# yassouali/pytorch-segmentation

Measured on NVIDIA H100. Metric: images/sec DeepLabV3+/ResNet101 513x513 train step (fwd+CE+bwd+SGD), higher is better.
Workload: dtype bf16

## Files before the change

### pytorch-segmentation_b200/csrc/seg_conv_tc.cu

```cuda
#include <cuda.h>
#include <mutex>
#include <stdlib.h>
#include "seg_common.cuh"
#include "seg_ptx.cuh"
#include "seg_sync.cuh"

namespace seg {
namespace tc {

using namespace ptx;

constexpr int BM = 128;
constexpr int BK = 64;
constexpr int A_BYTES = BM * 128;
constexpr int KIND_KK = 0, KIND_KM = 1, KIND_MM = 2;
constexpr int NTHREADS = 384;
constexpr int NCONS = 256;
constexpr int MAXT = 49;

struct TcParams {
  CUtensorMap mapA;
  CUtensorMap mapB;
  int M;
  int Ncols;
  int taps;
  int kchunks;
  int stride;
  int lower_h, lower_w;
  int PQ, Q;
  int x_im2col;
  int brows_per_tap;
  short tap_wt[MAXT];
  short tap_oh[MAXT];
  short tap_ow[MAXT];
  void* out;
  long long ldo;
  int out_dtype;
  float beta;
  const float* bias;
  double* stats;
  unsigned* stat_ticket;
  SyncDesc sync;
  int out_strided, out_H, out_W, osy, osx, opy, opx;
  int kblocks_total, kblocks_per_split;
  float* dw;
  int dw_K, dw_C;
  float* ws;
};

template <int BN>
struct Cfg {
  static constexpr int B_BYTES = BN * 128;
  static constexpr int STAGE_BYTES = A_BYTES + B_BYTES;
  static constexpr int STAGES = BN == 64 ? 6 : (BN == 128 ? 5 : 4);
  static constexpr int STAT_BYTES = 2 * 2 * BN * 4;
  static constexpr int SMEM = STAGES * STAGE_BYTES + STAT_BYTES + 1024  + 256 ;
  static_assert(STAGES * STAGE_BYTES >= BM * BN * 4, "staging tile must fit in the pipeline ring");
  static_assert(SMEM <= 227 * 1024, "shared memory per block");
};

__device__ __forceinline__ void row_to_coords(int m, int PQ, int Q, int stride, int lower_h, int lower_w, int& n, int& h,
                                              int& w) {
  n = m / PQ;
  int rem = m - n * PQ;
  int pp = rem / Q;
  int qq = rem - pp * Q;
  h = lower_h + pp * stride;
  w = lower_w + qq * stride;
}

template <int BN, int TA, int TB>
__device__ __forceinline__ void wgmma_tile(float* acc, uint64_t adesc, uint64_t bdesc, uint32_t accumulate) {
  if constexpr (BN == 64) wgmma_m64n64k16<TA, TB>(acc, adesc, bdesc, accumulate);
  else if constexpr (BN == 128) wgmma_m64n128k16<TA, TB>(acc, adesc, bdesc, accumulate);
  else wgmma_m64n256k16<TA, TB>(acc, adesc, bdesc, accumulate);
}

__device__ __forceinline__ void consumer_sync() { asm volatile("bar.sync 1, 256;" ::: "memory"); }

template <int BN, int KIND>
__global__ void __launch_bounds__(NTHREADS, 1) conv_gemm_tc(const __grid_constant__ TcParams p) {
  using C = Cfg<BN>;
  constexpr int STAGES = C::STAGES;
  extern __shared__ uint8_t smem_raw[];
  const uint32_t raw_addr = smem_u32(smem_raw);
  const uint32_t smem0 = (raw_addr + 1023u) & ~1023u;
  uint8_t* smem_gen = smem_raw + (smem0 - raw_addr);
  float* stat_sm = reinterpret_cast<float*>(smem_gen + STAGES * C::STAGE_BYTES);
  const uint32_t bar0 = smem0 + STAGES * C::STAGE_BYTES + C::STAT_BYTES;
  auto full_bar = [&](int s) { return bar0 + 8u * s; };
  auto empty_bar = [&](int s) { return bar0 + 8u * (STAGES + s); };
  volatile int* flag_sm = reinterpret_cast<volatile int*>(smem_gen + STAGES * C::STAGE_BYTES + C::STAT_BYTES + 8 * 2 * STAGES);

  const int m0 = blockIdx.x * BM;
  const int n0 = blockIdx.y * BN;

  int tap_mm = 0, kb_begin = 0, kb_end = 0, num_iters;
  if (KIND == KIND_MM) {
    tap_mm = blockIdx.z % p.taps;
    const int split = blockIdx.z / p.taps;
    kb_begin = split * p.kblocks_per_split;
    kb_end = min(kb_begin + p.kblocks_per_split, p.kblocks_total);
    num_iters = max(kb_end - kb_begin, 0);
  } else {
    num_iters = p.taps * p.kchunks;
  }

  if (threadIdx.x == 0) {
    prefetch_tmap(&p.mapA);
    prefetch_tmap(&p.mapB);
    for (int s = 0; s < STAGES; ++s) {
      mbar_init(full_bar(s), 1);
      mbar_init(empty_bar(s), 8);
    }
    fence_mbar_init();
  }
  __syncthreads();
  pdl_wait();

  if (threadIdx.x < 128) {
    if (threadIdx.x == 0 && num_iters > 0) {
      if (KIND != KIND_MM) {
        int n_img = 0, h0 = 0, w0 = 0;
        if (p.x_im2col) row_to_coords(m0, p.PQ, p.Q, p.stride, p.lower_h, p.lower_w, n_img, h0, w0);
        int it = 0;
        for (int tap = 0; tap < p.taps; ++tap) {
          const int wtap = p.tap_wt[tap];
          const uint16_t oh = (uint16_t)p.tap_oh[tap], ow = (uint16_t)p.tap_ow[tap];
          for (int kc = 0; kc < p.kchunks; ++kc, ++it) {
            const int st = it % STAGES;
            const uint32_t ph = (it / STAGES) & 1;
            mbar_wait_nocall(empty_bar(st), ph ^ 1u);
            const uint32_t a_dst = smem0 + st * C::STAGE_BYTES;
            const uint32_t b_dst = a_dst + A_BYTES;
            mbar_arrive_expect_tx(full_bar(st), C::STAGE_BYTES);
            if (p.x_im2col)
              tma_load_im2col_4d(a_dst, &p.mapA, full_bar(st), kc * BK, w0, h0, n_img, ow, oh);
            else
              tma_load_2d(a_dst, &p.mapA, full_bar(st), kc * BK, m0);
            if (KIND == KIND_KK) {
              tma_load_2d(b_dst, &p.mapB, full_bar(st), kc * BK, wtap * p.brows_per_tap + n0);
            } else {
#pragma unroll
              for (int j = 0; j < BN / 64; ++j)
                tma_load_2d(b_dst + j * 8192, &p.mapB, full_bar(st), n0 + j * 64, wtap * p.brows_per_tap + kc * BK);
            }
          }
        }
      } else {
        const uint16_t oh = (uint16_t)p.tap_oh[tap_mm], ow = (uint16_t)p.tap_ow[tap_mm];
        int it = 0;
        for (int kb = kb_begin; kb < kb_end; ++kb, ++it) {
          const int st = it % STAGES;
          const uint32_t ph = (it / STAGES) & 1;
          mbar_wait_nocall(empty_bar(st), ph ^ 1u);
          const uint32_t a_dst = smem0 + st * C::STAGE_BYTES;
          const uint32_t b_dst = a_dst + A_BYTES;
          const int pix0 = kb * BK;
          mbar_arrive_expect_tx(full_bar(st), C::STAGE_BYTES);
          tma_load_2d(a_dst, &p.mapA, full_bar(st), m0, pix0);
          tma_load_2d(a_dst + 8192, &p.mapA, full_bar(st), m0 + 64, pix0);
          if (p.x_im2col) {
            int n_img, h0, w0;
            row_to_coords(pix0, p.PQ, p.Q, p.stride, p.lower_h, p.lower_w, n_img, h0, w0);
#pragma unroll
            for (int j = 0; j < BN / 64; ++j)
              tma_load_im2col_4d(b_dst + j * 8192, &p.mapB, full_bar(st), n0 + j * 64, w0, h0, n_img, ow, oh);
          } else {
#pragma unroll
            for (int j = 0; j < BN / 64; ++j) tma_load_2d(b_dst + j * 8192, &p.mapB, full_bar(st), n0 + j * 64, pix0);
          }
        }
      }
    }
    return;
  }

  if (KIND == KIND_MM && num_iters == 0) return;
  const int ctid = threadIdx.x - 128;
  const int cw = ctid >> 7;
  const int warp = (ctid >> 5) & 3, lane = ctid & 31;
  float acc[BN / 2];
#pragma unroll
  for (int i = 0; i < BN / 2; ++i) acc[i] = 0.f;
  {
    constexpr int TA = (KIND == KIND_MM) ? 1 : 0;
    constexpr int TB = (KIND == KIND_KK) ? 0 : 1;
    for (int it = 0; it < num_iters; ++it) {
      const int st = it % STAGES;
      mbar_wait_nocall(full_bar(st), (it / STAGES) & 1);
      const uint32_t a_addr = smem0 + st * C::STAGE_BYTES + cw * 8192;
      const uint32_t b_addr = smem0 + st * C::STAGE_BYTES + A_BYTES;
      const uint64_t adesc0 = make_smem_desc_sw128(a_addr, TA ? 8192 : 16, 1024);
      const uint64_t bdesc0 = make_smem_desc_sw128(b_addr, TB ? 8192 : 16, 1024);
      wgmma_fence();
#pragma unroll
      for (int k = 0; k < BK / 16; ++k) {
        const uint64_t adesc = adesc0 + (uint64_t)(TA ? (k * 2048 >> 4) : (k * 32 >> 4));
        const uint64_t bdesc = bdesc0 + (uint64_t)(TB ? (k * 2048 >> 4) : (k * 32 >> 4));
        wgmma_tile<BN, TA, TB>(acc, adesc, bdesc, 1u);
      }
      wgmma_commit();
      wgmma_wait<1>();
      __syncwarp();
      if (it > 0 && lane == 0) mbar_arrive(empty_bar((it - 1) % STAGES));
    }
    wgmma_wait<0>();
  }
  consumer_sync();

  const bool out_f32 = (KIND == KIND_MM) || p.out_dtype != SEG_DT_BF16;
  const int esize = out_f32 ? 4 : 2;
  const int CPR = BN * esize / 16;
  const int swz = (CPR >= 32 ? 31 : CPR - 1);
  uint8_t* stage = smem_gen;
  const int ncols_tile = min(BN, p.Ncols - n0);
  {
    const int r0 = cw * 64 + warp * 16 + (lane >> 2);
#pragma unroll
    for (int j = 0; j < BN / 8; ++j) {
      const int col = j * 8 + 2 * (lane & 3);
      float b0 = 0.f, b1 = 0.f;
      if (KIND != KIND_MM && p.bias) {
        if (col < ncols_tile) b0 = __ldg(p.bias + n0 + col);
        if (col + 1 < ncols_tile) b1 = __ldg(p.bias + n0 + col + 1);
      }
#pragma unroll
      for (int h = 0; h < 2; ++h) {
        const int r = r0 + 8 * h;
        const float x0 = acc[4 * j + 2 * h] + b0, x1 = acc[4 * j + 2 * h + 1] + b1;
        const int byte = col * esize;
        uint8_t* dst = stage + (size_t)r * (BN * esize) + ((((byte >> 4) ^ (r & swz))) << 4) + (byte & 15);
        if (out_f32)
          *reinterpret_cast<float2*>(dst) = make_float2(x0, x1);
        else
          *reinterpret_cast<__nv_bfloat162*>(dst) = __floats2bfloat162_rn(x0, x1);
      }
    }
  }
  consumer_sync();

  if (KIND == KIND_MM) {
    float* base = p.ws ? p.ws + (size_t)(blockIdx.z / p.taps) * p.taps * p.dw_K * p.dw_C : p.dw;
    for (int idx = ctid; idx < BM * CPR; idx += NCONS) {
      const int tr = idx / CPR, c16 = idx - tr * CPR;
      const int row = m0 + tr, col0 = c16 * 4;
      if (row >= p.M || col0 >= ncols_tile) continue;
      const float4 v = *reinterpret_cast<const float4*>(stage + (size_t)tr * (BN * 4) + ((c16 ^ (tr & swz)) << 4));
      float* dst = base + ((size_t)tap_mm * p.dw_K + row) * p.dw_C + n0 + col0;
      const bool vec = col0 + 4 <= ncols_tile && ((reinterpret_cast<uintptr_t>(dst) & 15) == 0);
      const float a[4] = {v.x, v.y, v.z, v.w};
      if (p.ws) {
        if (vec)
          *reinterpret_cast<float4*>(dst) = v;
        else
          for (int i = 0; i < 4; ++i)
            if (col0 + i < ncols_tile) dst[i] = a[i];
      } else if (vec) {
        asm volatile("red.global.add.v4.f32 [%0], {%1, %2, %3, %4};" ::"l"(dst), "f"(v.x), "f"(v.y), "f"(v.z), "f"(v.w)
                     : "memory");
      } else {
        for (int i = 0; i < 4; ++i)
          if (col0 + i < ncols_tile) atomicAdd(dst + i, a[i]);
      }
    }
    return;
  }

  if (p.stats) {
    constexpr int NG = NCONS / BN, RPG = BM / NG;
    const int c = ctid % BN, g = ctid / BN;
    const int rend = min((g + 1) * RPG, p.M - m0);
    float s1 = 0.f, s2 = 0.f;
    const int byte = c * esize;
    for (int r = g * RPG; r < rend; ++r) {
      const uint8_t* src = stage + (size_t)r * (BN * esize) + ((((byte >> 4) ^ (r & swz))) << 4) + (byte & 15);
      const float x = out_f32 ? *reinterpret_cast<const float*>(src) : bf2f(*reinterpret_cast<const __nv_bfloat16*>(src));
      s1 += x;
      s2 = fmaf(x, x, s2);
    }
    stat_sm[(g * 2 + 0) * BN + c] = s1;
    stat_sm[(g * 2 + 1) * BN + c] = s2;
  }

  {
    const int nchunks = (ncols_tile * esize + 15) >> 4;
    const bool vec_ok = ((p.ldo * esize) & 15) == 0 && ((reinterpret_cast<uintptr_t>(p.out) + (size_t)n0 * esize) & 15) == 0;
    for (int idx = ctid; idx < BM * CPR; idx += NCONS) {
      const int tr = idx / CPR;
      const int c16 = idx - tr * CPR;
      if (c16 >= nchunks) continue;
      const int grow = m0 + tr;
      if (grow >= p.M) continue;
      long long pixel = grow;
      if (p.out_strided) {
        const int n = grow / p.PQ;
        const int rem = grow - n * p.PQ;
        const int i = rem / p.Q, j = rem - i * p.Q;
        pixel = ((long long)n * p.out_H + (i * p.osy + p.opy)) * p.out_W + (j * p.osx + p.opx);
      }
      const uint8_t* src = stage + (size_t)tr * (BN * esize) + ((c16 ^ (tr & swz)) << 4);
      uint8_t* dst = reinterpret_cast<uint8_t*>(p.out) + ((size_t)pixel * p.ldo + n0) * esize + ((size_t)c16 << 4);
      const int first_col = (c16 << 4) / esize;
      const bool full = first_col + 16 / esize <= ncols_tile;
      if (!out_f32) {
        bf16x8 val = *reinterpret_cast<const bf16x8*>(src);
        if (vec_ok && full) {
          if (p.beta != 0.f) {
            float a[8], b[8];
            unpack8(val, a);
            unpack8(*reinterpret_cast<const bf16x8*>(dst), b);
#pragma unroll
            for (int k = 0; k < 8; ++k) a[k] += p.beta * b[k];
            val = pack8(a);
          }
          *reinterpret_cast<bf16x8*>(dst) = val;
        } else {
          float a[8];
          unpack8(val, a);
          __nv_bfloat16* d = reinterpret_cast<__nv_bfloat16*>(dst);
          for (int k = 0; k < 8; ++k)
            if (first_col + k < ncols_tile) {
              float o = a[k];
              if (p.beta != 0.f) o += p.beta * bf2f(d[k]);
              d[k] = f2bf(o);
            }
        }
      } else {
        const float4 val = *reinterpret_cast<const float4*>(src);
        const float a[4] = {val.x, val.y, val.z, val.w};
        float* d = reinterpret_cast<float*>(dst);
        if (vec_ok && full && p.beta == 0.f) {
          *reinterpret_cast<float4*>(d) = val;
        } else {
          for (int k = 0; k < 4; ++k)
            if (first_col + k < ncols_tile) d[k] = (p.beta != 0.f) ? a[k] + p.beta * d[k] : a[k];
        }
      }
    }
  }
  if (num_iters > 0 && ctid == 0) pdl_trigger();

  if (p.stats) {
    constexpr int NG = NCONS / BN;
    consumer_sync();
    for (int c = ctid; c < ncols_tile; c += NCONS) {
      float a = 0.f, b = 0.f;
#pragma unroll
      for (int g = 0; g < NG; ++g) {
        a += stat_sm[(g * 2 + 0) * BN + c];
        b += stat_sm[(g * 2 + 1) * BN + c];
      }
      atomicAdd(p.stats + n0 + c, (double)a);
      atomicAdd(p.stats + p.Ncols + n0 + c, (double)b);
    }
    if (p.sync.world > 0)
      sync_push_when_last<false>(p.sync, p.stats, 2 * p.Ncols, p.stat_ticket, gridDim.x * gridDim.y, ctid, NCONS,
                          [] { asm volatile("bar.sync 1, 256;" ::: "memory"); }, flag_sm);
  }
}

typedef CUresult (*EncodeTiledFn)(CUtensorMap*, CUtensorMapDataType, cuuint32_t, void*, const cuuint64_t*,
                                  const cuuint64_t*, const cuuint32_t*, const cuuint32_t*, CUtensorMapInterleave,
                                  CUtensorMapSwizzle, CUtensorMapL2promotion, CUtensorMapFloatOOBfill);
typedef CUresult (*EncodeIm2colFn)(CUtensorMap*, CUtensorMapDataType, cuuint32_t, void*, const cuuint64_t*,
                                   const cuuint64_t*, const int*, const int*, cuuint32_t, cuuint32_t,
                                   const cuuint32_t*, CUtensorMapInterleave, CUtensorMapSwizzle,
                                   CUtensorMapL2promotion, CUtensorMapFloatOOBfill);
static EncodeTiledFn g_encode_tiled = nullptr;
static EncodeIm2colFn g_encode_im2col = nullptr;
static int g_driver_version = 0;

static int resolve_driver() {
  static std::once_flag once;
  static int status = 0;
  std::call_once(once, [] {
    void* f1 = nullptr;
    void* f2 = nullptr;
    cudaDriverEntryPointQueryResult q;
    if (cudaGetDriverEntryPoint("cuTensorMapEncodeTiled", &f1, cudaEnableDefault, &q) != cudaSuccess || !f1) status = 1;
    if (cudaGetDriverEntryPoint("cuTensorMapEncodeIm2col", &f2, cudaEnableDefault, &q) != cudaSuccess || !f2) status = 1;
    g_encode_tiled = (EncodeTiledFn)f1;
    g_encode_im2col = (EncodeIm2colFn)f2;
    cudaDriverGetVersion(&g_driver_version);
  });
  if (status) set_error("cannot resolve cuTensorMapEncode* driver entry points");
  return status;
}

static int make_map_2d(CUtensorMap* m, const void* ptr, int64_t rows, int64_t cols, int64_t ld, int box_rows) {
  if (resolve_driver()) return 1;
  SEG_REQUIRE((reinterpret_cast<uintptr_t>(ptr) & 15) == 0, "TMA: base pointer not 16-byte aligned");
  SEG_REQUIRE(ld % 8 == 0, "TMA: row pitch %lld not a multiple of 8 elements", (long long)ld);
  cuuint64_t dims[2] = {(cuuint64_t)cols, (cuuint64_t)rows};
  cuuint64_t strides[1] = {(cuuint64_t)ld * 2};
  cuuint32_t box[2] = {64, (cuuint32_t)box_rows};
  cuuint32_t es[2] = {1, 1};
  CUresult r = g_encode_tiled(m, CU_TENSOR_MAP_DATA_TYPE_BFLOAT16, 2, const_cast<void*>(ptr), dims, strides, box, es,
                              CU_TENSOR_MAP_INTERLEAVE_NONE, CU_TENSOR_MAP_SWIZZLE_128B,
                              CU_TENSOR_MAP_L2_PROMOTION_L2_256B, CU_TENSOR_MAP_FLOAT_OOB_FILL_NONE);
  SEG_REQUIRE(r == CUDA_SUCCESS, "cuTensorMapEncodeTiled failed (%d) rows=%lld cols=%lld ld=%lld box_rows=%d", (int)r,
              (long long)rows, (long long)cols, (long long)ld, box_rows);
  return 0;
}

static int make_map_im2col(CUtensorMap* m, const void* ptr, int N, int H, int W, int C, int64_t ld, int lower_w,
                           int lower_h, int upper_w, int upper_h, int stride, int pixels) {
  if (resolve_driver()) return 1;
  SEG_REQUIRE((reinterpret_cast<uintptr_t>(ptr) & 15) == 0, "TMA: base pointer not 16-byte aligned");
  SEG_REQUIRE(ld % 8 == 0, "TMA: channel pitch %lld not a multiple of 8", (long long)ld);
  SEG_REQUIRE(lower_w >= -128 && upper_w >= -128 && lower_w <= 127 && upper_w <= 127 && lower_h >= -128 &&
                  upper_h >= -128 && lower_h <= 127 && upper_h <= 127,
              "im2col corner out of range");
  cuuint64_t dims[4] = {(cuuint64_t)C, (cuuint64_t)W, (cuuint64_t)H, (cuuint64_t)N};
  cuuint64_t strides[3] = {(cuuint64_t)ld * 2, (cuuint64_t)W * ld * 2, (cuuint64_t)H * W * ld * 2};
  int lo[2] = {lower_w, lower_h};
  int up[2] = {upper_w, upper_h};
  cuuint32_t es[4] = {1, (cuuint32_t)stride, (cuuint32_t)stride, 1};
  CUresult r = g_encode_im2col(m, CU_TENSOR_MAP_DATA_TYPE_BFLOAT16, 4, const_cast<void*>(ptr), dims, strides, lo, up,
                               64, (cuuint32_t)pixels, es, CU_TENSOR_MAP_INTERLEAVE_NONE, CU_TENSOR_MAP_SWIZZLE_128B,
                               CU_TENSOR_MAP_L2_PROMOTION_L2_256B, CU_TENSOR_MAP_FLOAT_OOB_FILL_NONE);
  SEG_REQUIRE(r == CUDA_SUCCESS,
              "cuTensorMapEncodeIm2col failed (%d) N=%d H=%d W=%d C=%d ld=%lld lo=(%d,%d) up=(%d,%d) s=%d", (int)r, N, H,
              W, C, (long long)ld, lower_w, lower_h, upper_w, upper_h, stride);
  if (g_driver_version <= 13010) {
    const uint64_t bytes = (uint64_t)N * H * W * ld * 2;
    if (bytes < 131072) reinterpret_cast<uint64_t*>(m)[1] &= ~(1ull << 21);
  }
  return 0;
}

template <int BN, int KIND>
static int launch_kernel(const TcParams& p, dim3 grid, cudaStream_t stream) {
  static bool attr_set = false;
  auto kfn = conv_gemm_tc<BN, KIND>;
  if (!attr_set) {
    cudaError_t e = cudaFuncSetAttribute(kfn, cudaFuncAttributeMaxDynamicSharedMemorySize, Cfg<BN>::SMEM);
    SEG_REQUIRE(e == cudaSuccess, "cudaFuncSetAttribute(smem=%d): %s", Cfg<BN>::SMEM, cudaGetErrorString(e));
    attr_set = true;
  }
  launch_pdl(kfn, grid, dim3(NTHREADS), (size_t)Cfg<BN>::SMEM, stream, p);
  return check_launch("conv_gemm_tc");
}

template <int KIND>
static int launch_bn(int bn, const TcParams& p, dim3 grid, cudaStream_t stream) {
  switch (bn) {
    case 64: return launch_kernel<64, KIND>(p, grid, stream);
    case 128: return launch_kernel<128, KIND>(p, grid, stream);
    case 256: return launch_kernel<256, KIND>(p, grid, stream);
  }
  set_error("bad BN %d", bn);
  return 1;
}

static int pick_bn(int ncols) {
  if (ncols <= 64) return 64;
  if (ncols < 256) return 128;
  const int waste = ceil_div(ncols, 256) * 256 - ncols;
  return waste < 128 ? 256 : 128;
}

bool supported(const seg_conv_desc* d) {
  if (d->C % 8 != 0 || d->ldx % 8 != 0) return false;
  if (d->R != d->S) return false;
  if (d->R * d->S > MAXT) return false;
  if (d->pad > 127 || d->dil * (d->R - 1) - d->pad > 127 || d->dil * (d->R - 1) - d->pad < -127) return false;
  if (d->stride > 8) return false;
  return true;
}

static bool is_pointwise(const seg_conv_desc* d) { return d->R == 1 && d->S == 1 && d->stride == 1 && d->pad == 0; }

int conv_fwd(const seg_conv_desc* d, const void* x, const void* w, void* y, int y_dtype, const float* bias, float beta,
             double* stats, unsigned* stat_ticket, const SyncDesc* sync, cudaStream_t stream) {
  SEG_REQUIRE(supported(d), "wgmma conv fwd: unsupported shape (C=%d ldx=%d R=%d pad=%d dil=%d)", d->C, d->ldx, d->R,
              d->pad, d->dil);
  TcParams p;
  memset(&p, 0, sizeof(p));
  const int64_t M = (int64_t)d->N * d->P * d->Q;
  SEG_REQUIRE(M < (1ll << 31), "M too large");
  p.M = (int)M;
  p.Ncols = d->K;
  p.taps = d->R * d->S;
  for (int t = 0; t < p.taps; ++t) {
    p.tap_wt[t] = (short)t;
    p.tap_oh[t] = (short)((t / d->S) * d->dil);
    p.tap_ow[t] = (short)((t % d->S) * d->dil);
  }
  p.kchunks = ceil_div(d->C, BK);
  p.stride = d->stride;
  p.lower_h = p.lower_w = -d->pad;
  p.PQ = d->P * d->Q;
  p.Q = d->Q;
  p.brows_per_tap = d->K;
  p.out = y;
  p.ldo = d->ldy;
  p.out_dtype = y_dtype;
  p.beta = beta;
  p.bias = bias;
  p.stats = stats;
  p.stat_ticket = stat_ticket;
  if (sync && stats) {
    SEG_REQUIRE(stat_ticket != nullptr, "conv fwd: SyncBN needs a zeroed ticket word");
    SEG_REQUIRE(4 * d->K <= sync->n_max, "conv fwd: 2*K = %d fp64 statistics exceed the SyncBN buffer (%d floats)", 2 * d->K, sync->n_max);
    p.sync = *sync;
  }
  const int64_t m_tiles = ceil_div64(M, BM);
  const int bn = pick_bn(d->K);
  if (is_pointwise(d)) {
    p.x_im2col = 0;
    if (make_map_2d(&p.mapA, x, M, d->C, d->ldx, BM)) return 1;
  } else {
    p.x_im2col = 1;
    const int upper = d->pad - (d->R - 1) * d->dil;
    if (make_map_im2col(&p.mapA, x, d->N, d->H, d->W, d->C, d->ldx, -d->pad, -d->pad, upper, upper, d->stride, BM)) return 1;
  }
  if (make_map_2d(&p.mapB, w, (int64_t)p.taps * d->K, d->C, d->C, bn)) return 1;
  dim3 grid((unsigned)m_tiles, (unsigned)ceil_div(d->K, bn), 1);
  return launch_bn<KIND_KK>(bn, p, grid, stream);
}

static int floordiv(int a, int b) { return (a >= 0) ? a / b : -((-a + b - 1) / b); }

int conv_dgrad(const seg_conv_desc* d, const void* dy, const void* w, void* dx, float beta, cudaStream_t stream) {
  SEG_REQUIRE(supported(d) && d->ldy % 8 == 0, "wgmma conv dgrad: unsupported shape (stride=%d K=%d ldy=%d)", d->stride,
              d->K, d->ldy);
  const int s = d->stride;
  const int bn = pick_bn(d->C);
  for (int py = 0; py < s; ++py) {
    for (int px = 0; px < s; ++px) {
      const int Hs = (d->H - py + s - 1) / s, Ws = (d->W - px + s - 1) / s;
      if (Hs <= 0 || Ws <= 0) continue;
      TcParams p;
      memset(&p, 0, sizeof(p));
      int rh[8], oh[8], nh = 0, rw[8], ow[8], nw = 0;
      for (int r = 0; r < d->R; ++r) {
        const int num = py + d->pad - r * d->dil;
        if (((num % s) + s) % s == 0) { rh[nh] = r; oh[nh] = floordiv(num, s); ++nh; }
      }
      for (int q = 0; q < d->S; ++q) {
        const int num = px + d->pad - q * d->dil;
        if (((num % s) + s) % s == 0) { rw[nw] = q; ow[nw] = floordiv(num, s); ++nw; }
      }
      int min_oh = 0, min_ow = 0;
      for (int i = 0; i < nh; ++i) min_oh = (i == 0) ? oh[i] : min(min_oh, oh[i]);
      for (int i = 0; i < nw; ++i) min_ow = (i == 0) ? ow[i] : min(min_ow, ow[i]);
      p.taps = nh * nw;
      for (int i = 0; i < nh; ++i)
        for (int j = 0; j < nw; ++j) {
          const int t = i * nw + j;
          p.tap_wt[t] = (short)(rh[i] * d->S + rw[j]);
          p.tap_oh[t] = (short)(oh[i] - min_oh);
          p.tap_ow[t] = (short)(ow[j] - min_ow);
        }
      const int64_t M = (int64_t)d->N * Hs * Ws;
      SEG_REQUIRE(M < (1ll << 31), "M too large");
      p.M = (int)M;
      p.Ncols = d->C;
      p.kchunks = ceil_div(d->K, BK);
      p.stride = 1;
      p.lower_h = min_oh;
      p.lower_w = min_ow;
      p.PQ = Hs * Ws;
      p.Q = Ws;
      p.brows_per_tap = d->K;
      p.out = dx;
      p.ldo = d->ldx;
      p.out_dtype = SEG_DT_BF16;
      p.beta = beta;
      if (s > 1) {
        p.out_strided = 1;
        p.out_H = d->H;
        p.out_W = d->W;
        p.osy = p.osx = s;
        p.opy = py;
        p.opx = px;
      }
      const int64_t m_tiles = ceil_div64(M, BM);
      if (p.taps > 0) {
        const bool plain = (s == 1 && is_pointwise(d));
        if (plain) {
          p.x_im2col = 0;
          if (make_map_2d(&p.mapA, dy, M, d->K, d->ldy, BM)) return 1;
        } else {
          p.x_im2col = 1;
          const int upper_h = Hs - d->P + min_oh, upper_w = Ws - d->Q + min_ow;
          if (make_map_im2col(&p.mapA, dy, d->N, d->P, d->Q, d->K, d->ldy, min_ow, min_oh, upper_w, upper_h, 1, BM)) return 1;
        }
        if (make_map_2d(&p.mapB, w, (int64_t)d->R * d->S * d->K, d->C, d->C, 64)) return 1;
      } else {
        if (beta != 0.f) continue;
        if (make_map_2d(&p.mapA, w, (int64_t)d->R * d->S * d->K, d->C, d->C, BM)) return 1;
        if (make_map_2d(&p.mapB, w, (int64_t)d->R * d->S * d->K, d->C, d->C, 64)) return 1;
      }
      dim3 grid((unsigned)m_tiles, (unsigned)ceil_div(d->C, bn), 1);
      if (launch_bn<KIND_KM>(bn, p, grid, stream)) return 1;
    }
  }
  return 0;
}

__global__ void wgrad_split_reduce_kernel(const float* __restrict__ ws, int splits, int64_t n, float* __restrict__ dw) {
  for (int64_t i = blockIdx.x * (int64_t)blockDim.x + threadIdx.x; i < n; i += (int64_t)gridDim.x * blockDim.x) {
    float acc = ws[i];
    for (int s = 1; s < splits; ++s) acc += ws[(size_t)s * n + i];
    dw[i] += acc;
  }
}

static void wgrad_plan(const seg_conv_desc* d, int& bn, int& splits, int& kblocks_per_split) {
  const bool wide = d->R * d->S >= 9 && d->C >= 256 && d->C % 256 == 0;
  bn = (d->C <= 64) ? 64 : (wide ? 256 : 128);
  const int kblocks_total = (int)ceil_div64((int64_t)d->N * d->P * d->Q, BK);
  const int tiles = ceil_div(d->K, BM) * ceil_div(d->C, bn) * d->R * d->S;
  splits = max(1, num_sms() / tiles);
  splits = min(splits, kblocks_total);
  splits = min(splits, 1024);
  kblocks_per_split = ceil_div(kblocks_total, splits);
  splits = ceil_div(kblocks_total, kblocks_per_split);
}

int64_t wgrad_workspace_floats(const seg_conv_desc* d) {
  if (!supported(d)) return 0;
  int bn, splits, kps;
  wgrad_plan(d, bn, splits, kps);
  return splits > 1 ? (int64_t)splits * d->R * d->S * d->K * d->C : 0;
}

int conv_wgrad(const seg_conv_desc* d, const void* dy, const void* x, float* dw, float* ws, cudaStream_t stream) {
  SEG_REQUIRE(supported(d) && d->ldy % 8 == 0, "wgmma conv wgrad: unsupported shape");
  TcParams p;
  memset(&p, 0, sizeof(p));
  const int64_t npix = (int64_t)d->N * d->P * d->Q;
  SEG_REQUIRE(npix < (1ll << 31), "too many pixels");
  p.M = d->K;
  p.Ncols = d->C;
  p.taps = d->R * d->S;
  for (int t = 0; t < p.taps; ++t) {
    p.tap_wt[t] = (short)t;
    p.tap_oh[t] = (short)((t / d->S) * d->dil);
    p.tap_ow[t] = (short)((t % d->S) * d->dil);
  }
  p.stride = d->stride;
  p.lower_h = p.lower_w = -d->pad;
  p.PQ = d->P * d->Q;
  p.Q = d->Q;
  p.dw = dw;
  p.dw_K = d->K;
  p.dw_C = d->C;
  p.kblocks_total = (int)ceil_div64(npix, BK);
  int bn, splits;
  wgrad_plan(d, bn, splits, p.kblocks_per_split);
  SEG_REQUIRE(splits == 1 || ws != nullptr, "wgmma conv wgrad: %d k-splits need the workspace (seg_conv2d_wgrad_workspace_floats)", splits);
  SEG_REQUIRE((int64_t)(splits - 1) * p.kblocks_per_split < p.kblocks_total, "wgmma conv wgrad: split %d has no k-blocks", splits - 1);
  if (splits > 1) p.ws = ws;
  if (make_map_2d(&p.mapA, dy, npix, d->K, d->ldy, 64)) return 1;
  if (is_pointwise(d)) {
    p.x_im2col = 0;
    if (make_map_2d(&p.mapB, x, npix, d->C, d->ldx, 64)) return 1;
  } else {
    p.x_im2col = 1;
    const int upper = d->pad - (d->R - 1) * d->dil;
    if (make_map_im2col(&p.mapB, x, d->N, d->H, d->W, d->C, d->ldx, -d->pad, -d->pad, upper, upper, d->stride, 64)) return 1;
  }
  SEG_REQUIRE((unsigned)(p.taps * splits) <= 65535u, "wgrad grid.z too large");
  dim3 grid((unsigned)ceil_div(d->K, BM), (unsigned)ceil_div(d->C, bn), (unsigned)(p.taps * splits));
  if (launch_bn<KIND_MM>(bn, p, grid, stream)) return 1;
  if (splits == 1) return 0;
  const int64_t n = (int64_t)p.taps * d->K * d->C;
  wgrad_split_reduce_kernel<<<(unsigned)std::min<int64_t>(ceil_div64(n, 256), (int64_t)num_sms() * 8), 256, 0, stream>>>(ws, splits, n, dw);
  return check_launch("wgrad_split_reduce");
}

}
}
```

### pytorch-segmentation_b200/csrc/seg_ptx.cuh

```cuda
#pragma once
#include <cuda.h>
#include <stdint.h>

namespace seg {
namespace ptx {

__device__ __forceinline__ uint32_t smem_u32(const void* p) { return (uint32_t)__cvta_generic_to_shared(p); }

__device__ __forceinline__ void mbar_init(uint32_t bar, uint32_t count) {
  asm volatile("mbarrier.init.shared::cta.b64 [%0], %1;" ::"r"(bar), "r"(count) : "memory");
}
__device__ __forceinline__ void fence_mbar_init() {
  asm volatile("fence.mbarrier_init.release.cluster;" ::: "memory");
}
__device__ __forceinline__ void fence_proxy_async() {
  asm volatile("fence.proxy.async.shared::cta;" ::: "memory");
}
__device__ __forceinline__ void mbar_arrive(uint32_t bar) {
  asm volatile("mbarrier.arrive.shared::cta.b64 _, [%0];" ::"r"(bar) : "memory");
}
__device__ __forceinline__ void mbar_arrive_expect_tx(uint32_t bar, uint32_t bytes) {
  asm volatile("mbarrier.arrive.expect_tx.shared::cta.b64 _, [%0], %1;" ::"r"(bar), "r"(bytes) : "memory");
}
__device__ __forceinline__ uint32_t mbar_try_wait(uint32_t bar, uint32_t parity) {
  uint32_t ok;
  asm volatile(
      "{\n\t.reg .pred p;\n\t"
      "mbarrier.try_wait.parity.shared::cta.b64 p, [%1], %2;\n\t"
      "selp.u32 %0, 1, 0, p;\n\t}"
      : "=r"(ok)
      : "r"(bar), "r"(parity)
      : "memory");
  return ok;
}
__device__ __forceinline__ void mbar_wait(uint32_t bar, uint32_t parity) {
  if (mbar_try_wait(bar, parity)) return;
  long long t0 = clock64();
  while (!mbar_try_wait(bar, parity)) {
    if (clock64() - t0 > 4000000000ll) {
      printf("seg_b200: mbarrier wait timeout (block %d,%d,%d thread %d bar %u parity %u)\n", blockIdx.x,
             blockIdx.y, blockIdx.z, threadIdx.x, bar, parity);
      __trap();
    }
  }
}

__device__ __forceinline__ void mbar_wait_nocall(uint32_t bar, uint32_t parity) {
  if (mbar_try_wait(bar, parity)) return;
  long long t0 = clock64();
  while (!mbar_try_wait(bar, parity))
    if (clock64() - t0 > 4000000000ll) __trap();
}

__device__ __forceinline__ void prefetch_tmap(const CUtensorMap* m) {
  asm volatile("prefetch.tensormap [%0];" ::"l"(reinterpret_cast<uint64_t>(m)) : "memory");
}
__device__ __forceinline__ void tma_load_2d(uint32_t dst, const CUtensorMap* m, uint32_t bar, int c0, int c1) {
  asm volatile(
      "cp.async.bulk.tensor.2d.shared::cluster.global.mbarrier::complete_tx::bytes [%0], [%1, {%3, %4}], [%2];" ::"r"(dst),
      "l"(reinterpret_cast<uint64_t>(m)), "r"(bar), "r"(c0), "r"(c1)
      : "memory");
}
__device__ __forceinline__ void tma_load_im2col_4d(uint32_t dst, const CUtensorMap* m, uint32_t bar, int c, int w,
                                                   int h, int n, uint16_t off_w, uint16_t off_h) {
  asm volatile(
      "cp.async.bulk.tensor.4d.shared::cluster.global.im2col.mbarrier::complete_tx::bytes [%0], [%1, {%3, %4, %5, "
      "%6}], [%2], {%7, %8};" ::"r"(dst),
      "l"(reinterpret_cast<uint64_t>(m)), "r"(bar), "r"(c), "r"(w), "r"(h), "r"(n), "h"(off_w), "h"(off_h)
      : "memory");
}

__device__ __forceinline__ void wgmma_fence() { asm volatile("wgmma.fence.sync.aligned;" ::: "memory"); }
__device__ __forceinline__ void wgmma_commit() { asm volatile("wgmma.commit_group.sync.aligned;" ::: "memory"); }
template <int N>
__device__ __forceinline__ void wgmma_wait() { asm volatile("wgmma.wait_group.sync.aligned %0;" ::"n"(N) : "memory"); }

__device__ __forceinline__ uint64_t make_smem_desc_sw128(uint32_t smem_addr, uint32_t lbo_bytes, uint32_t sbo_bytes) {
  uint64_t d = 0;
  d |= (uint64_t)((smem_addr & 0x3FFFFu) >> 4);
  d |= (uint64_t)((lbo_bytes >> 4) & 0x3FFFu) << 16;
  d |= (uint64_t)((sbo_bytes >> 4) & 0x3FFFu) << 32;
  d |= (uint64_t)1 << 62;
  return d;
}

template <int TA, int TB>
__device__ __forceinline__ void wgmma_m64n64k16(float* d, uint64_t adesc, uint64_t bdesc, uint32_t accumulate) {
  asm volatile(
      "{\n\t.reg .pred p;\n\tsetp.ne.b32 p, %34, 0;\n\t"
      "wgmma.mma_async.sync.aligned.m64n64k16.f32.bf16.bf16 "
      "{%0, %1, %2, %3, %4, %5, %6, %7, %8, %9, %10, %11, %12, %13, %14, %15, %16, %17, %18, %19, %20, %21, %22, %23, %24, %25, %26, %27, %28, %29, %30, %31}, %32, %33, p, 1, 1, %35, %36;\n\t}"
      : "+f"(d[0]), "+f"(d[1]), "+f"(d[2]), "+f"(d[3]), "+f"(d[4]), "+f"(d[5]), "+f"(d[6]), "+f"(d[7]), "+f"(d[8]), "+f"(d[9]), "+f"(d[10]), "+f"(d[11]), "+f"(d[12]), "+f"(d[13]), "+f"(d[14]), "+f"(d[15]), "+f"(d[16]), "+f"(d[17]), "+f"(d[18]), "+f"(d[19]), "+f"(d[20]), "+f"(d[21]), "+f"(d[22]), "+f"(d[23]), "+f"(d[24]), "+f"(d[25]), "+f"(d[26]), "+f"(d[27]), "+f"(d[28]), "+f"(d[29]), "+f"(d[30]), "+f"(d[31])
      : "l"(adesc), "l"(bdesc), "r"(accumulate), "n"(TA), "n"(TB)
      : "memory");
}

template <int TA, int TB>
__device__ __forceinline__ void wgmma_m64n128k16(float* d, uint64_t adesc, uint64_t bdesc, uint32_t accumulate) {
  asm volatile(
      "{\n\t.reg .pred p;\n\tsetp.ne.b32 p, %66, 0;\n\t"
      "wgmma.mma_async.sync.aligned.m64n128k16.f32.bf16.bf16 "
      "{%0, %1, %2, %3, %4, %5, %6, %7, %8, %9, %10, %11, %12, %13, %14, %15, %16, %17, %18, %19, %20, %21, %22, %23, %24, %25, %26, %27, %28, %29, %30, %31, %32, %33, %34, %35, %36, %37, %38, %39, %40, %41, %42, %43, %44, %45, %46, %47, %48, %49, %50, %51, %52, %53, %54, %55, %56, %57, %58, %59, %60, %61, %62, %63}, %64, %65, p, 1, 1, %67, %68;\n\t}"
      : "+f"(d[0]), "+f"(d[1]), "+f"(d[2]), "+f"(d[3]), "+f"(d[4]), "+f"(d[5]), "+f"(d[6]), "+f"(d[7]), "+f"(d[8]), "+f"(d[9]), "+f"(d[10]), "+f"(d[11]), "+f"(d[12]), "+f"(d[13]), "+f"(d[14]), "+f"(d[15]), "+f"(d[16]), "+f"(d[17]), "+f"(d[18]), "+f"(d[19]), "+f"(d[20]), "+f"(d[21]), "+f"(d[22]), "+f"(d[23]), "+f"(d[24]), "+f"(d[25]), "+f"(d[26]), "+f"(d[27]), "+f"(d[28]), "+f"(d[29]), "+f"(d[30]), "+f"(d[31]), "+f"(d[32]), "+f"(d[33]), "+f"(d[34]), "+f"(d[35]), "+f"(d[36]), "+f"(d[37]), "+f"(d[38]), "+f"(d[39]), "+f"(d[40]), "+f"(d[41]), "+f"(d[42]), "+f"(d[43]), "+f"(d[44]), "+f"(d[45]), "+f"(d[46]), "+f"(d[47]), "+f"(d[48]), "+f"(d[49]), "+f"(d[50]), "+f"(d[51]), "+f"(d[52]), "+f"(d[53]), "+f"(d[54]), "+f"(d[55]), "+f"(d[56]), "+f"(d[57]), "+f"(d[58]), "+f"(d[59]), "+f"(d[60]), "+f"(d[61]), "+f"(d[62]), "+f"(d[63])
      : "l"(adesc), "l"(bdesc), "r"(accumulate), "n"(TA), "n"(TB)
      : "memory");
}

template <int TA, int TB>
__device__ __forceinline__ void wgmma_m64n256k16(float* d, uint64_t adesc, uint64_t bdesc, uint32_t accumulate) {
  asm volatile(
      "{\n\t.reg .pred p;\n\tsetp.ne.b32 p, %130, 0;\n\t"
      "wgmma.mma_async.sync.aligned.m64n256k16.f32.bf16.bf16 "
      "{%0, %1, %2, %3, %4, %5, %6, %7, %8, %9, %10, %11, %12, %13, %14, %15, %16, %17, %18, %19, %20, %21, %22, %23, %24, %25, %26, %27, %28, %29, %30, %31, %32, %33, %34, %35, %36, %37, %38, %39, %40, %41, %42, %43, %44, %45, %46, %47, %48, %49, %50, %51, %52, %53, %54, %55, %56, %57, %58, %59, %60, %61, %62, %63, %64, %65, %66, %67, %68, %69, %70, %71, %72, %73, %74, %75, %76, %77, %78, %79, %80, %81, %82, %83, %84, %85, %86, %87, %88, %89, %90, %91, %92, %93, %94, %95, %96, %97, %98, %99, %100, %101, %102, %103, %104, %105, %106, %107, %108, %109, %110, %111, %112, %113, %114, %115, %116, %117, %118, %119, %120, %121, %122, %123, %124, %125, %126, %127}, %128, %129, p, 1, 1, %131, %132;\n\t}"
      : "+f"(d[0]), "+f"(d[1]), "+f"(d[2]), "+f"(d[3]), "+f"(d[4]), "+f"(d[5]), "+f"(d[6]), "+f"(d[7]), "+f"(d[8]), "+f"(d[9]), "+f"(d[10]), "+f"(d[11]), "+f"(d[12]), "+f"(d[13]), "+f"(d[14]), "+f"(d[15]), "+f"(d[16]), "+f"(d[17]), "+f"(d[18]), "+f"(d[19]), "+f"(d[20]), "+f"(d[21]), "+f"(d[22]), "+f"(d[23]), "+f"(d[24]), "+f"(d[25]), "+f"(d[26]), "+f"(d[27]), "+f"(d[28]), "+f"(d[29]), "+f"(d[30]), "+f"(d[31]), "+f"(d[32]), "+f"(d[33]), "+f"(d[34]), "+f"(d[35]), "+f"(d[36]), "+f"(d[37]), "+f"(d[38]), "+f"(d[39]), "+f"(d[40]), "+f"(d[41]), "+f"(d[42]), "+f"(d[43]), "+f"(d[44]), "+f"(d[45]), "+f"(d[46]), "+f"(d[47]), "+f"(d[48]), "+f"(d[49]), "+f"(d[50]), "+f"(d[51]), "+f"(d[52]), "+f"(d[53]), "+f"(d[54]), "+f"(d[55]), "+f"(d[56]), "+f"(d[57]), "+f"(d[58]), "+f"(d[59]), "+f"(d[60]), "+f"(d[61]), "+f"(d[62]), "+f"(d[63]), "+f"(d[64]), "+f"(d[65]), "+f"(d[66]), "+f"(d[67]), "+f"(d[68]), "+f"(d[69]), "+f"(d[70]), "+f"(d[71]), "+f"(d[72]), "+f"(d[73]), "+f"(d[74]), "+f"(d[75]), "+f"(d[76]), "+f"(d[77]), "+f"(d[78]), "+f"(d[79]), "+f"(d[80]), "+f"(d[81]), "+f"(d[82]), "+f"(d[83]), "+f"(d[84]), "+f"(d[85]), "+f"(d[86]), "+f"(d[87]), "+f"(d[88]), "+f"(d[89]), "+f"(d[90]), "+f"(d[91]), "+f"(d[92]), "+f"(d[93]), "+f"(d[94]), "+f"(d[95]), "+f"(d[96]), "+f"(d[97]), "+f"(d[98]), "+f"(d[99]), "+f"(d[100]), "+f"(d[101]), "+f"(d[102]), "+f"(d[103]), "+f"(d[104]), "+f"(d[105]), "+f"(d[106]), "+f"(d[107]), "+f"(d[108]), "+f"(d[109]), "+f"(d[110]), "+f"(d[111]), "+f"(d[112]), "+f"(d[113]), "+f"(d[114]), "+f"(d[115]), "+f"(d[116]), "+f"(d[117]), "+f"(d[118]), "+f"(d[119]), "+f"(d[120]), "+f"(d[121]), "+f"(d[122]), "+f"(d[123]), "+f"(d[124]), "+f"(d[125]), "+f"(d[126]), "+f"(d[127])
      : "l"(adesc), "l"(bdesc), "r"(accumulate), "n"(TA), "n"(TB)
      : "memory");
}

}
}
```

Baseline: 332.4.

## Use persistent ping-pong warp-specialized kernel for conv fprop and dgrad

Replaces the one-tile-per-block conv GEMM for forward and data-gradient convolutions with a persistent kernel sized to the SM count. In it, two consumer warpgroups alternate output tiles (ping-pong), using named barriers to order mainloops so one group's epilogue overlaps the other's MMA. Each warpgroup now computes a full 128-row tile with two accumulators, and registers are rebalanced with setmaxnreg. BN is restricted to 64/128 with fewer stages, and BN statistics grouping is parameterized. The aim is to hide epilogue and stats cost and reduce launch/tail overhead, at the cost of more register pressure and smaller tiles for wide layers.

Result: faster. 352.4, median of 6 (+6.0%).

```diff
diff --git a/pytorch-segmentation_b200/csrc/seg_conv_tc.cu b/pytorch-segmentation_b200/csrc/seg_conv_tc.cu
--- a/pytorch-segmentation_b200/csrc/seg_conv_tc.cu
+++ b/pytorch-segmentation_b200/csrc/seg_conv_tc.cu
@@ -13,10 +13,14 @@
 constexpr int BM = 128;
 constexpr int BK = 64;
 constexpr int A_BYTES = BM * 128;
-constexpr int KIND_KK = 0, KIND_KM = 1, KIND_MM = 2;
+constexpr int KIND_KK = 0, KIND_KM = 1;
 constexpr int NTHREADS = 384;
 constexpr int NCONS = 256;
 constexpr int MAXT = 49;
+
+constexpr int BAR_CONSUMERS = 1;
+constexpr int BAR_ORDER = 2;
+constexpr int BAR_WG = 4;
 
 struct TcParams {
   CUtensorMap mapA;
@@ -39,24 +43,15 @@
   float beta;
   const float* bias;
   double* stats;
+  int stat_rows;
   unsigned* stat_ticket;
   SyncDesc sync;
   int out_strided, out_H, out_W, osy, osx, opy, opx;
+  int n_tiles, tiles;
   int kblocks_total, kblocks_per_split;
   float* dw;
   int dw_K, dw_C;
   float* ws;
-};
-
-template <int BN>
-struct Cfg {
-  static constexpr int B_BYTES = BN * 128;
-  static constexpr int STAGE_BYTES = A_BYTES + B_BYTES;
-  static constexpr int STAGES = BN == 64 ? 6 : (BN == 128 ? 5 : 4);
-  static constexpr int STAT_BYTES = 2 * 2 * BN * 4;
-  static constexpr int SMEM = STAGES * STAGE_BYTES + STAT_BYTES + 1024  + 256 ;
-  static_assert(STAGES * STAGE_BYTES >= BM * BN * 4, "staging tile must fit in the pipeline ring");
-  static_assert(SMEM <= 227 * 1024, "shared memory per block");
 };
 
 __device__ __forceinline__ void row_to_coords(int m, int PQ, int Q, int stride, int lower_h, int lower_w, int& n, int& h,
@@ -76,35 +71,312 @@
   else wgmma_m64n256k16<TA, TB>(acc, adesc, bdesc, accumulate);
 }
 
-__device__ __forceinline__ void consumer_sync() { asm volatile("bar.sync 1, 256;" ::: "memory"); }
-
 template <int BN, int KIND>
-__global__ void __launch_bounds__(NTHREADS, 1) conv_gemm_tc(const __grid_constant__ TcParams p) {
+__device__ __forceinline__ void load_kblock(const TcParams& p, uint32_t a_dst, uint32_t bar, int kc, int wtap, uint16_t oh,
+                                            uint16_t ow, int n_img, int h0, int w0, int m0, int n0) {
+  const uint32_t b_dst = a_dst + A_BYTES;
+  if (p.x_im2col)
+    tma_load_im2col_4d(a_dst, &p.mapA, bar, kc * BK, w0, h0, n_img, ow, oh);
+  else
+    tma_load_2d(a_dst, &p.mapA, bar, kc * BK, m0);
+  if (KIND == KIND_KK) {
+    tma_load_2d(b_dst, &p.mapB, bar, kc * BK, wtap * p.brows_per_tap + n0);
+  } else {
+#pragma unroll
+    for (int j = 0; j < BN / 64; ++j)
+      tma_load_2d(b_dst + j * 8192, &p.mapB, bar, n0 + j * 64, wtap * p.brows_per_tap + kc * BK);
+  }
+}
+
+template <int BN>
+__device__ __forceinline__ void stage_acc(const float* acc, const float* acc1, uint8_t* stage, int rbase, int warp, int lane,
+                                          const float* bias, bool out_f32) {
+  const int esize = out_f32 ? 4 : 2;
+  const int CPR = BN * esize / 16;
+  const int swz = (CPR >= 32 ? 31 : CPR - 1);
+  const int r0 = rbase + warp * 16 + (lane >> 2);
+#pragma unroll
+  for (int j = 0; j < BN / 8; ++j) {
+    const int col = j * 8 + 2 * (lane & 3);
+    float b0 = 0.f, b1 = 0.f;
+    if (bias) {
+      b0 = bias[col];
+      b1 = bias[col + 1];
+    }
+#pragma unroll
+    for (int h = 0; h < 4; ++h) {
+      if (h >= 2 && !acc1) break;
+      const float* a = h < 2 ? acc : acc1;
+      const int r = r0 + 8 * (h & 1) + 32 * (h & 2);
+      const float x0 = a[4 * j + 2 * (h & 1)] + b0, x1 = a[4 * j + 2 * (h & 1) + 1] + b1;
+      const int byte = col * esize;
+      uint8_t* dst = stage + (size_t)r * (BN * esize) + ((((byte >> 4) ^ (r & swz))) << 4) + (byte & 15);
+      if (out_f32)
+        *reinterpret_cast<float2*>(dst) = make_float2(x0, x1);
+      else
+        *reinterpret_cast<__nv_bfloat162*>(dst) = __floats2bfloat162_rn(x0, x1);
+    }
+  }
+}
+
+
+template <int BN>
+struct PPCfg {
+  static_assert(BN == 64 || BN == 128, "ping-pong tile width");
+  static constexpr int B_BYTES = BN * 128;
+  static constexpr int STAGE_BYTES = A_BYTES + B_BYTES;
+  static constexpr int STAGES = BN == 64 ? 6 : 4;
+  static constexpr int RING = STAGES * STAGE_BYTES;
+  static constexpr int STG_BYTES = BM * 256;
+  static constexpr int MAXG = BM / 32;
+  static constexpr int STAT_BYTES = MAXG * 2 * BN * 4 + BN * 4;
+  static constexpr int SMEM = RING + 2 * (STG_BYTES + STAT_BYTES) + 1024  + 256 ;
+  static_assert(16 * STAGES + 8 <= 256, "barrier area");
+  static_assert(SMEM <= 227 * 1024, "shared memory per block");
+};
+
+template <int BN, int KIND>
+__global__ void __launch_bounds__(NTHREADS, 1) conv_gemm_pp(const __grid_constant__ TcParams p) {
+  using C = PPCfg<BN>;
+  constexpr int STAGES = C::STAGES;
+  extern __shared__ uint8_t smem_raw[];
+  const uint32_t raw_addr = smem_u32(smem_raw);
+  const uint32_t smem0 = (raw_addr + 1023u) & ~1023u;
+  uint8_t* smem_gen = smem_raw + (smem0 - raw_addr);
+  const uint32_t bar0 = smem0 + C::RING + 2 * (C::STG_BYTES + C::STAT_BYTES);
+  auto full_bar = [&](int s) { return bar0 + 8u * s; };
+  auto empty_bar = [&](int s) { return bar0 + 8u * (STAGES + s); };
+  volatile int* flag_sm = reinterpret_cast<volatile int*>(smem_gen + (bar0 - smem0) + 16 * STAGES);
+
+  const int num_iters = p.taps * p.kchunks;
+  const int grid = gridDim.x;
+  const int ntiles = (p.tiles - (int)blockIdx.x + grid - 1) / grid;
+
+  if (threadIdx.x == 0) {
+    prefetch_tmap(&p.mapA);
+    prefetch_tmap(&p.mapB);
+    for (int s = 0; s < STAGES; ++s) {
+      mbar_init(full_bar(s), 1);
+      mbar_init(empty_bar(s), 4);
+    }
+    fence_mbar_init();
+  }
+  __syncthreads();
+  pdl_wait();
+
+  if (threadIdx.x < 128) {
+    setmaxnreg_dec<40>();
+    if (threadIdx.x == 0 && num_iters > 0) {
+      int it = 0;
+      for (int j = 0; j < ntiles; ++j) {
+        const int t = blockIdx.x + j * grid;
+        const int m0 = (t / p.n_tiles) * BM, n0 = (t % p.n_tiles) * BN;
+        int n_img = 0, h0 = 0, w0 = 0;
+        if (p.x_im2col) row_to_coords(m0, p.PQ, p.Q, p.stride, p.lower_h, p.lower_w, n_img, h0, w0);
+        for (int tap = 0; tap < p.taps; ++tap) {
+          const int wtap = p.tap_wt[tap];
+          const uint16_t oh = (uint16_t)p.tap_oh[tap], ow = (uint16_t)p.tap_ow[tap];
+          for (int kc = 0; kc < p.kchunks; ++kc, ++it) {
+            const int st = it % STAGES;
+            mbar_wait_nocall(empty_bar(st), ((it / STAGES) & 1) ^ 1u);
+            mbar_arrive_expect_tx(full_bar(st), C::STAGE_BYTES);
+            load_kblock<BN, KIND>(p, smem0 + st * C::STAGE_BYTES, full_bar(st), kc, wtap, oh, ow, n_img, h0, w0, m0, n0);
+          }
+        }
+      }
+    }
+    return;
+  }
+
+  setmaxnreg_inc<232>();
+  const int cw = (threadIdx.x - 128) >> 7;
+  const int tid = threadIdx.x & 127;
+  const int warp = tid >> 5, lane = tid & 31;
+  uint8_t* stage = smem_gen + C::RING + cw * C::STG_BYTES;
+  float* stat_sm = reinterpret_cast<float*>(smem_gen + C::RING + 2 * C::STG_BYTES + cw * C::STAT_BYTES);
+  float* bias_sm = stat_sm + C::MAXG * 2 * BN;
+  const bool out_f32 = p.out_dtype != SEG_DT_BF16;
+  const int esize = out_f32 ? 4 : 2;
+  const int CPR = BN * esize / 16;
+  const int swz = (CPR >= 32 ? 31 : CPR - 1);
+  auto wg_sync = [&] { named_sync(BAR_WG + cw, 128); };
+
+  for (int j = cw; j < ntiles; j += 2) {
+    const int t = blockIdx.x + j * grid;
+    const int m0 = (t / p.n_tiles) * BM, n0 = (t % p.n_tiles) * BN;
+    float acc0[BN / 2], acc1[BN / 2];
+#pragma unroll
+    for (int i = 0; i < BN / 2; ++i) acc0[i] = acc1[i] = 0.f;
+
+    if (j > 0) named_sync(BAR_ORDER + cw, NCONS);
+    {
+      constexpr int TB = (KIND == KIND_KK) ? 0 : 1;
+      const int it0 = j * num_iters;
+      for (int i = 0; i < num_iters; ++i) {
+        const int it = it0 + i;
+        const int st = it % STAGES;
+        mbar_wait_nocall(full_bar(st), (it / STAGES) & 1);
+        const uint32_t a_addr = smem0 + st * C::STAGE_BYTES;
+        const uint32_t b_addr = a_addr + A_BYTES;
+        const uint64_t adesc0 = make_smem_desc_sw128(a_addr, 16, 1024);
+        const uint64_t adesc1 = make_smem_desc_sw128(a_addr + 8192, 16, 1024);
+        const uint64_t bdesc0 = make_smem_desc_sw128(b_addr, TB ? 8192 : 16, 1024);
+        wgmma_fence();
+#pragma unroll
+        for (int k = 0; k < BK / 16; ++k) {
+          const uint64_t bdesc = bdesc0 + (uint64_t)(TB ? (k * 2048 >> 4) : (k * 32 >> 4));
+          wgmma_tile<BN, 0, TB>(acc0, adesc0 + (uint64_t)(k * 32 >> 4), bdesc, 1u);
+          wgmma_tile<BN, 0, TB>(acc1, adesc1 + (uint64_t)(k * 32 >> 4), bdesc, 1u);
+        }
+        wgmma_commit();
+        wgmma_wait<1>();
+        __syncwarp();
+        if (i > 0 && lane == 0) mbar_arrive(empty_bar((it - 1) % STAGES));
+      }
+      if (j + 1 < ntiles) named_arrive(BAR_ORDER + (cw ^ 1), NCONS);
+      wgmma_wait<0>();
+      __syncwarp();
+      if (num_iters > 0 && lane == 0) mbar_arrive(empty_bar((it0 + num_iters - 1) % STAGES));
+    }
+
+    const int ncols_tile = min(BN, p.Ncols - n0);
+    if (p.bias && tid < BN) bias_sm[tid] = tid < ncols_tile ? __ldg(p.bias + n0 + tid) : 0.f;
+    wg_sync();
+    stage_acc<BN>(acc0, acc1, stage, 0, warp, lane, p.bias ? bias_sm : nullptr, out_f32);
+    wg_sync();
+
+    const int ngroups = BM / p.stat_rows;
+    if (p.stats) {
+      const int parts = min(128 / BN, ngroups);
+      const int rpp = BM / parts;
+      const int c = tid % BN, part = tid / BN;
+      const int rvalid = min(BM, p.M - m0);
+      if (part < parts) {
+        const int byte = c * esize;
+        int g = part * rpp / p.stat_rows;
+        for (int rg = part * rpp; rg < (part + 1) * rpp; rg += p.stat_rows, ++g) {
+          float s1 = 0.f, s2 = 0.f;
+          const int rend = min(rg + p.stat_rows, rvalid);
+          for (int r = rg; r < rend; ++r) {
+            const uint8_t* src = stage + (size_t)r * (BN * esize) + ((((byte >> 4) ^ (r & swz))) << 4) + (byte & 15);
+            const float x = out_f32 ? *reinterpret_cast<const float*>(src) : bf2f(*reinterpret_cast<const __nv_bfloat16*>(src));
+            s1 += x;
+            s2 = fmaf(x, x, s2);
+          }
+          stat_sm[(g * 2 + 0) * BN + c] = s1;
+          stat_sm[(g * 2 + 1) * BN + c] = s2;
+        }
+      }
+    }
+
+    {
+      const int nchunks = (ncols_tile * esize + 15) >> 4;
+      const bool vec_ok = ((p.ldo * esize) & 15) == 0 && ((reinterpret_cast<uintptr_t>(p.out) + (size_t)n0 * esize) & 15) == 0;
+      for (int idx = tid; idx < BM * CPR; idx += 128) {
+        const int tr = idx / CPR;
+        const int c16 = idx - tr * CPR;
+        if (c16 >= nchunks) continue;
+        const int grow = m0 + tr;
+        if (grow >= p.M) continue;
+        long long pixel = grow;
+        if (p.out_strided) {
+          const int n = grow / p.PQ;
+          const int rem = grow - n * p.PQ;
+          const int i = rem / p.Q, jj = rem - i * p.Q;
+          pixel = ((long long)n * p.out_H + (i * p.osy + p.opy)) * p.out_W + (jj * p.osx + p.opx);
+        }
+        const uint8_t* src = stage + (size_t)tr * (BN * esize) + ((c16 ^ (tr & swz)) << 4);
+        uint8_t* dst = reinterpret_cast<uint8_t*>(p.out) + ((size_t)pixel * p.ldo + n0) * esize + ((size_t)c16 << 4);
+        const int first_col = (c16 << 4) / esize;
+        const bool full = first_col + 16 / esize <= ncols_tile;
+        if (!out_f32) {
+          bf16x8 val = *reinterpret_cast<const bf16x8*>(src);
+          if (vec_ok && full) {
+            if (p.beta != 0.f) {
+              float a[8], b[8];
+              unpack8(val, a);
+              unpack8(*reinterpret_cast<const bf16x8*>(dst), b);
+#pragma unroll
+              for (int k = 0; k < 8; ++k) a[k] += p.beta * b[k];
+              val = pack8(a);
+            }
+            *reinterpret_cast<bf16x8*>(dst) = val;
+          } else {
+            float a[8];
+            unpack8(val, a);
+            __nv_bfloat16* d = reinterpret_cast<__nv_bfloat16*>(dst);
+            for (int k = 0; k < 8; ++k)
+              if (first_col + k < ncols_tile) {
+                float o = a[k];
+                if (p.beta != 0.f) o += p.beta * bf2f(d[k]);
+                d[k] = f2bf(o);
+              }
+          }
+        } else {
+          const float4 val = *reinterpret_cast<const float4*>(src);
+          const float a[4] = {val.x, val.y, val.z, val.w};
+          float* d = reinterpret_cast<float*>(dst);
+          if (vec_ok && full && p.beta == 0.f) {
+            *reinterpret_cast<float4*>(d) = val;
+          } else {
+            for (int k = 0; k < 4; ++k)
+              if (first_col + k < ncols_tile) d[k] = (p.beta != 0.f) ? a[k] + p.beta * d[k] : a[k];
+          }
+        }
+      }
+    }
+    if (j == ntiles - 1 && tid == 0) pdl_trigger();
+
+    if (p.stats) {
+      wg_sync();
+      if (tid < ncols_tile) {
+        float a = 0.f, b = 0.f;
+        for (int g = 0; g < ngroups; ++g) {
+          a += stat_sm[(g * 2 + 0) * BN + tid];
+          b += stat_sm[(g * 2 + 1) * BN + tid];
+        }
+        atomicAdd(p.stats + n0 + tid, (double)a);
+        atomicAdd(p.stats + p.Ncols + n0 + tid, (double)b);
+      }
+    }
+  }
+
+  if (p.stats && p.sync.world > 0)
+    sync_push_when_last<false>(p.sync, p.stats, 2 * p.Ncols, p.stat_ticket, gridDim.x, threadIdx.x - 128, NCONS,
+                               [] { named_sync(BAR_CONSUMERS, NCONS); }, flag_sm);
+}
+
+
+template <int BN>
+struct Cfg {
+  static constexpr int B_BYTES = BN * 128;
+  static constexpr int STAGE_BYTES = A_BYTES + B_BYTES;
+  static constexpr int STAGES = BN == 64 ? 6 : (BN == 128 ? 5 : 4);
+  static constexpr int SMEM = STAGES * STAGE_BYTES + 1024  + 256 ;
+  static_assert(STAGES * STAGE_BYTES >= BM * BN * 4, "staging tile must fit in the pipeline ring");
+  static_assert(SMEM <= 227 * 1024, "shared memory per block");
+};
+
+template <int BN>
+__global__ void __launch_bounds__(NTHREADS, 1) conv_gemm_wgrad(const __grid_constant__ TcParams p) {
   using C = Cfg<BN>;
   constexpr int STAGES = C::STAGES;
   extern __shared__ uint8_t smem_raw[];
   const uint32_t raw_addr = smem_u32(smem_raw);
   const uint32_t smem0 = (raw_addr + 1023u) & ~1023u;
   uint8_t* smem_gen = smem_raw + (smem0 - raw_addr);
-  float* stat_sm = reinterpret_cast<float*>(smem_gen + STAGES * C::STAGE_BYTES);
-  const uint32_t bar0 = smem0 + STAGES * C::STAGE_BYTES + C::STAT_BYTES;
+  const uint32_t bar0 = smem0 + STAGES * C::STAGE_BYTES;
   auto full_bar = [&](int s) { return bar0 + 8u * s; };
   auto empty_bar = [&](int s) { return bar0 + 8u * (STAGES + s); };
-  volatile int* flag_sm = reinterpret_cast<volatile int*>(smem_gen + STAGES * C::STAGE_BYTES + C::STAT_BYTES + 8 * 2 * STAGES);
 
   const int m0 = blockIdx.x * BM;
   const int n0 = blockIdx.y * BN;
 
-  int tap_mm = 0, kb_begin = 0, kb_end = 0, num_iters;
-  if (KIND == KIND_MM) {
-    tap_mm = blockIdx.z % p.taps;
-    const int split = blockIdx.z / p.taps;
-    kb_begin = split * p.kblocks_per_split;
-    kb_end = min(kb_begin + p.kblocks_per_split, p.kblocks_total);
-    num_iters = max(kb_end - kb_begin, 0);
-  } else {
-    num_iters = p.taps * p.kchunks;
-  }
+  const int tap_mm = blockIdx.z % p.taps;
+  const int split = blockIdx.z / p.taps;
+  const int kb_begin = split * p.kblocks_per_split;
+  const int kb_end = min(kb_begin + p.kblocks_per_split, p.kblocks_total);
+  const int num_iters = max(kb_end - kb_begin, 0);
 
   if (threadIdx.x == 0) {
     prefetch_tmap(&p.mapA);
@@ -120,243 +392,88 @@
 
   if (threadIdx.x < 128) {
     if (threadIdx.x == 0 && num_iters > 0) {
-      if (KIND != KIND_MM) {
-        int n_img = 0, h0 = 0, w0 = 0;
-        if (p.x_im2col) row_to_coords(m0, p.PQ, p.Q, p.stride, p.lower_h, p.lower_w, n_img, h0, w0);
-        int it = 0;
-        for (int tap = 0; tap < p.taps; ++tap) {
-          const int wtap = p.tap_wt[tap];
-          const uint16_t oh = (uint16_t)p.tap_oh[tap], ow = (uint16_t)p.tap_ow[tap];
-          for (int kc = 0; kc < p.kchunks; ++kc, ++it) {
-            const int st = it % STAGES;
-            const uint32_t ph = (it / STAGES) & 1;
-            mbar_wait_nocall(empty_bar(st), ph ^ 1u);
-            const uint32_t a_dst = smem0 + st * C::STAGE_BYTES;
-            const uint32_t b_dst = a_dst + A_BYTES;
-            mbar_arrive_expect_tx(full_bar(st), C::STAGE_BYTES);
-            if (p.x_im2col)
-              tma_load_im2col_4d(a_dst, &p.mapA, full_bar(st), kc * BK, w0, h0, n_img, ow, oh);
-            else
-              tma_load_2d(a_dst, &p.mapA, full_bar(st), kc * BK, m0);
-            if (KIND == KIND_KK) {
-              tma_load_2d(b_dst, &p.mapB, full_bar(st), kc * BK, wtap * p.brows_per_tap + n0);
-            } else {
-#pragma unroll
-              for (int j = 0; j < BN / 64; ++j)
-                tma_load_2d(b_dst + j * 8192, &p.mapB, full_bar(st), n0 + j * 64, wtap * p.brows_per_tap + kc * BK);
-            }
-          }
+      const uint16_t oh = (uint16_t)p.tap_oh[tap_mm], ow = (uint16_t)p.tap_ow[tap_mm];
+      int it = 0;
+      for (int kb = kb_begin; kb < kb_end; ++kb, ++it) {
+        const int st = it % STAGES;
+        const uint32_t ph = (it / STAGES) & 1;
+        mbar_wait_nocall(empty_bar(st), ph ^ 1u);
+        const uint32_t a_dst = smem0 + st * C::STAGE_BYTES;
+        const uint32_t b_dst = a_dst + A_BYTES;
+        const int pix0 = kb * BK;
+        mbar_arrive_expect_tx(full_bar(st), C::STAGE_BYTES);
+        tma_load_2d(a_dst, &p.mapA, full_bar(st), m0, pix0);
+        tma_load_2d(a_dst + 8192, &p.mapA, full_bar(st), m0 + 64, pix0);
+        if (p.x_im2col) {
+          int n_img, h0, w0;
+          row_to_coords(pix0, p.PQ, p.Q, p.stride, p.lower_h, p.lower_w, n_img, h0, w0);
+#pragma unroll
+          for (int j = 0; j < BN / 64; ++j)
+            tma_load_im2col_4d(b_dst + j * 8192, &p.mapB, full_bar(st), n0 + j * 64, w0, h0, n_img, ow, oh);
+        } else {
+#pragma unroll
+          for (int j = 0; j < BN / 64; ++j) tma_load_2d(b_dst + j * 8192, &p.mapB, full_bar(st), n0 + j * 64, pix0);
         }
-      } else {
-        const uint16_t oh = (uint16_t)p.tap_oh[tap_mm], ow = (uint16_t)p.tap_ow[tap_mm];
-        int it = 0;
-        for (int kb = kb_begin; kb < kb_end; ++kb, ++it) {
-          const int st = it % STAGES;
-          const uint32_t ph = (it / STAGES) & 1;
-          mbar_wait_nocall(empty_bar(st), ph ^ 1u);
-          const uint32_t a_dst = smem0 + st * C::STAGE_BYTES;
-          const uint32_t b_dst = a_dst + A_BYTES;
-          const int pix0 = kb * BK;
-          mbar_arrive_expect_tx(full_bar(st), C::STAGE_BYTES);
-          tma_load_2d(a_dst, &p.mapA, full_bar(st), m0, pix0);
-          tma_load_2d(a_dst + 8192, &p.mapA, full_bar(st), m0 + 64, pix0);
-          if (p.x_im2col) {
-            int n_img, h0, w0;
-            row_to_coords(pix0, p.PQ, p.Q, p.stride, p.lower_h, p.lower_w, n_img, h0, w0);
-#pragma unroll
-            for (int j = 0; j < BN / 64; ++j)
-              tma_load_im2col_4d(b_dst + j * 8192, &p.mapB, full_bar(st), n0 + j * 64, w0, h0, n_img, ow, oh);
-          } else {
-#pragma unroll
-            for (int j = 0; j < BN / 64; ++j) tma_load_2d(b_dst + j * 8192, &p.mapB, full_bar(st), n0 + j * 64, pix0);
-          }
-        }
       }
     }
     return;
   }
 
-  if (KIND == KIND_MM && num_iters == 0) return;
+  if (num_iters == 0) return;
   const int ctid = threadIdx.x - 128;
   const int cw = ctid >> 7;
   const int warp = (ctid >> 5) & 3, lane = ctid & 31;
   float acc[BN / 2];
 #pragma unroll
   for (int i = 0; i < BN / 2; ++i) acc[i] = 0.f;
-  {
-    constexpr int TA = (KIND == KIND_MM) ? 1 : 0;
-    constexpr int TB = (KIND == KIND_KK) ? 0 : 1;
-    for (int it = 0; it < num_iters; ++it) {
-      const int st = it % STAGES;
-      mbar_wait_nocall(full_bar(st), (it / STAGES) & 1);
-      const uint32_t a_addr = smem0 + st * C::STAGE_BYTES + cw * 8192;
-      const uint32_t b_addr = smem0 + st * C::STAGE_BYTES + A_BYTES;
-      const uint64_t adesc0 = make_smem_desc_sw128(a_addr, TA ? 8192 : 16, 1024);
-      const uint64_t bdesc0 = make_smem_desc_sw128(b_addr, TB ? 8192 : 16, 1024);
-      wgmma_fence();
-#pragma unroll
-      for (int k = 0; k < BK / 16; ++k) {
-        const uint64_t adesc = adesc0 + (uint64_t)(TA ? (k * 2048 >> 4) : (k * 32 >> 4));
-        const uint64_t bdesc = bdesc0 + (uint64_t)(TB ? (k * 2048 >> 4) : (k * 32 >> 4));
-        wgmma_tile<BN, TA, TB>(acc, adesc, bdesc, 1u);
-      }
-      wgmma_commit();
-      wgmma_wait<1>();
-      __syncwarp();
-      if (it > 0 && lane == 0) mbar_arrive(empty_bar((it - 1) % STAGES));
-    }
-    wgmma_wait<0>();
-  }
-  consumer_sync();
-
-  const bool out_f32 = (KIND == KIND_MM) || p.out_dtype != SEG_DT_BF16;
-  const int esize = out_f32 ? 4 : 2;
-  const int CPR = BN * esize / 16;
-  const int swz = (CPR >= 32 ? 31 : CPR - 1);
+  for (int it = 0; it < num_iters; ++it) {
+    const int st = it % STAGES;
+    mbar_wait_nocall(full_bar(st), (it / STAGES) & 1);
+    const uint32_t a_addr = smem0 + st * C::STAGE_BYTES + cw * 8192;
+    const uint32_t b_addr = smem0 + st * C::STAGE_BYTES + A_BYTES;
+    const uint64_t adesc0 = make_smem_desc_sw128(a_addr, 8192, 1024);
+    const uint64_t bdesc0 = make_smem_desc_sw128(b_addr, 8192, 1024);
+    wgmma_fence();
+#pragma unroll
+    for (int k = 0; k < BK / 16; ++k)
+      wgmma_tile<BN, 1, 1>(acc, adesc0 + (uint64_t)(k * 2048 >> 4), bdesc0 + (uint64_t)(k * 2048 >> 4), 1u);
+    wgmma_commit();
+    wgmma_wait<1>();
+    __syncwarp();
+    if (it > 0 && lane == 0) mbar_arrive(empty_bar((it - 1) % STAGES));
+  }
+  wgmma_wait<0>();
+  named_sync(BAR_CONSUMERS, NCONS);
+
   uint8_t* stage = smem_gen;
   const int ncols_tile = min(BN, p.Ncols - n0);
-  {
-    const int r0 = cw * 64 + warp * 16 + (lane >> 2);
-#pragma unroll
-    for (int j = 0; j < BN / 8; ++j) {
-      const int col = j * 8 + 2 * (lane & 3);
-      float b0 = 0.f, b1 = 0.f;
-      if (KIND != KIND_MM && p.bias) {
-        if (col < ncols_tile) b0 = __ldg(p.bias + n0 + col);
-        if (col + 1 < ncols_tile) b1 = __ldg(p.bias + n0 + col + 1);
-      }
-#pragma unroll
-      for (int h = 0; h < 2; ++h) {
-        const int r = r0 + 8 * h;
-        const float x0 = acc[4 * j + 2 * h] + b0, x1 = acc[4 * j + 2 * h + 1] + b1;
-        const int byte = col * esize;
-        uint8_t* dst = stage + (size_t)r * (BN * esize) + ((((byte >> 4) ^ (r & swz))) << 4) + (byte & 15);
-        if (out_f32)
-          *reinterpret_cast<float2*>(dst) = make_float2(x0, x1);
-        else
-          *reinterpret_cast<__nv_bfloat162*>(dst) = __floats2bfloat162_rn(x0, x1);
-      }
-    }
-  }
-  consumer_sync();
-
-  if (KIND == KIND_MM) {
-    float* base = p.ws ? p.ws + (size_t)(blockIdx.z / p.taps) * p.taps * p.dw_K * p.dw_C : p.dw;
-    for (int idx = ctid; idx < BM * CPR; idx += NCONS) {
-      const int tr = idx / CPR, c16 = idx - tr * CPR;
-      const int row = m0 + tr, col0 = c16 * 4;
-      if (row >= p.M || col0 >= ncols_tile) continue;
-      const float4 v = *reinterpret_cast<const float4*>(stage + (size_t)tr * (BN * 4) + ((c16 ^ (tr & swz)) << 4));
-      float* dst = base + ((size_t)tap_mm * p.dw_K + row) * p.dw_C + n0 + col0;
-      const bool vec = col0 + 4 <= ncols_tile && ((reinterpret_cast<uintptr_t>(dst) & 15) == 0);
-      const float a[4] = {v.x, v.y, v.z, v.w};
-      if (p.ws) {
-        if (vec)
-          *reinterpret_cast<float4*>(dst) = v;
-        else
-          for (int i = 0; i < 4; ++i)
-            if (col0 + i < ncols_tile) dst[i] = a[i];
-      } else if (vec) {
-        asm volatile("red.global.add.v4.f32 [%0], {%1, %2, %3, %4};" ::"l"(dst), "f"(v.x), "f"(v.y), "f"(v.z), "f"(v.w)
-                     : "memory");
-      } else {
+  stage_acc<BN>(acc, nullptr, stage, cw * 64, warp, lane, nullptr, true);
+  named_sync(BAR_CONSUMERS, NCONS);
+
+  const int CPR = BN * 4 / 16;
+  const int swz = (CPR >= 32 ? 31 : CPR - 1);
+  float* base = p.ws ? p.ws + (size_t)split * p.taps * p.dw_K * p.dw_C : p.dw;
+  for (int idx = ctid; idx < BM * CPR; idx += NCONS) {
+    const int tr = idx / CPR, c16 = idx - tr * CPR;
+    const int row = m0 + tr, col0 = c16 * 4;
+    if (row >= p.M || col0 >= ncols_tile) continue;
+    const float4 v = *reinterpret_cast<const float4*>(stage + (size_t)tr * (BN * 4) + ((c16 ^ (tr & swz)) << 4));
+    float* dst = base + ((size_t)tap_mm * p.dw_K + row) * p.dw_C + n0 + col0;
+    const bool vec = col0 + 4 <= ncols_tile && ((reinterpret_cast<uintptr_t>(dst) & 15) == 0);
+    const float a[4] = {v.x, v.y, v.z, v.w};
+    if (p.ws) {
+      if (vec)
+        *reinterpret_cast<float4*>(dst) = v;
+      else
         for (int i = 0; i < 4; ++i)
-          if (col0 + i < ncols_tile) atomicAdd(dst + i, a[i]);
-      }
-    }
-    return;
-  }
-
-  if (p.stats) {
-    constexpr int NG = NCONS / BN, RPG = BM / NG;
-    const int c = ctid % BN, g = ctid / BN;
-    const int rend = min((g + 1) * RPG, p.M - m0);
-    float s1 = 0.f, s2 = 0.f;
-    const int byte = c * esize;
-    for (int r = g * RPG; r < rend; ++r) {
-      const uint8_t* src = stage + (size_t)r * (BN * esize) + ((((byte >> 4) ^ (r & swz))) << 4) + (byte & 15);
-      const float x = out_f32 ? *reinterpret_cast<const float*>(src) : bf2f(*reinterpret_cast<const __nv_bfloat16*>(src));
-      s1 += x;
-      s2 = fmaf(x, x, s2);
-    }
-    stat_sm[(g * 2 + 0) * BN + c] = s1;
-    stat_sm[(g * 2 + 1) * BN + c] = s2;
-  }
-
-  {
-    const int nchunks = (ncols_tile * esize + 15) >> 4;
-    const bool vec_ok = ((p.ldo * esize) & 15) == 0 && ((reinterpret_cast<uintptr_t>(p.out) + (size_t)n0 * esize) & 15) == 0;
-    for (int idx = ctid; idx < BM * CPR; idx += NCONS) {
-      const int tr = idx / CPR;
-      const int c16 = idx - tr * CPR;
-      if (c16 >= nchunks) continue;
-      const int grow = m0 + tr;
-      if (grow >= p.M) continue;
-      long long pixel = grow;
-      if (p.out_strided) {
-        const int n = grow / p.PQ;
-        const int rem = grow - n * p.PQ;
-        const int i = rem / p.Q, j = rem - i * p.Q;
-        pixel = ((long long)n * p.out_H + (i * p.osy + p.opy)) * p.out_W + (j * p.osx + p.opx);
-      }
-      const uint8_t* src = stage + (size_t)tr * (BN * esize) + ((c16 ^ (tr & swz)) << 4);
-      uint8_t* dst = reinterpret_cast<uint8_t*>(p.out) + ((size_t)pixel * p.ldo + n0) * esize + ((size_t)c16 << 4);
-      const int first_col = (c16 << 4) / esize;
-      const bool full = first_col + 16 / esize <= ncols_tile;
-      if (!out_f32) {
-        bf16x8 val = *reinterpret_cast<const bf16x8*>(src);
-        if (vec_ok && full) {
-          if (p.beta != 0.f) {
-            float a[8], b[8];
-            unpack8(val, a);
-            unpack8(*reinterpret_cast<const bf16x8*>(dst), b);
-#pragma unroll
-            for (int k = 0; k < 8; ++k) a[k] += p.beta * b[k];
-            val = pack8(a);
-          }
-          *reinterpret_cast<bf16x8*>(dst) = val;
-        } else {
-          float a[8];
-          unpack8(val, a);
-          __nv_bfloat16* d = reinterpret_cast<__nv_bfloat16*>(dst);
-          for (int k = 0; k < 8; ++k)
-            if (first_col + k < ncols_tile) {
-              float o = a[k];
-              if (p.beta != 0.f) o += p.beta * bf2f(d[k]);
-              d[k] = f2bf(o);
-            }
-        }
-      } else {
-        const float4 val = *reinterpret_cast<const float4*>(src);
-        const float a[4] = {val.x, val.y, val.z, val.w};
-        float* d = reinterpret_cast<float*>(dst);
-        if (vec_ok && full && p.beta == 0.f) {
-          *reinterpret_cast<float4*>(d) = val;
-        } else {
-          for (int k = 0; k < 4; ++k)
-            if (first_col + k < ncols_tile) d[k] = (p.beta != 0.f) ? a[k] + p.beta * d[k] : a[k];
-        }
-      }
-    }
-  }
-  if (num_iters > 0 && ctid == 0) pdl_trigger();
-
-  if (p.stats) {
-    constexpr int NG = NCONS / BN;
-    consumer_sync();
-    for (int c = ctid; c < ncols_tile; c += NCONS) {
-      float a = 0.f, b = 0.f;
-#pragma unroll
-      for (int g = 0; g < NG; ++g) {
-        a += stat_sm[(g * 2 + 0) * BN + c];
-        b += stat_sm[(g * 2 + 1) * BN + c];
-      }
-      atomicAdd(p.stats + n0 + c, (double)a);
-      atomicAdd(p.stats + p.Ncols + n0 + c, (double)b);
-    }
-    if (p.sync.world > 0)
-      sync_push_when_last<false>(p.sync, p.stats, 2 * p.Ncols, p.stat_ticket, gridDim.x * gridDim.y, ctid, NCONS,
-                          [] { asm volatile("bar.sync 1, 256;" ::: "memory"); }, flag_sm);
+          if (col0 + i < ncols_tile) dst[i] = a[i];
+    } else if (vec) {
+      asm volatile("red.global.add.v4.f32 [%0], {%1, %2, %3, %4};" ::"l"(dst), "f"(v.x), "f"(v.y), "f"(v.z), "f"(v.w)
+                   : "memory");
+    } else {
+      for (int i = 0; i < 4; ++i)
+        if (col0 + i < ncols_tile) atomicAdd(dst + i, a[i]);
+    }
   }
 }
 
@@ -431,34 +548,63 @@
 }
 
 template <int BN, int KIND>
-static int launch_kernel(const TcParams& p, dim3 grid, cudaStream_t stream) {
+static int launch_pp(TcParams& p, cudaStream_t stream) {
   static bool attr_set = false;
-  auto kfn = conv_gemm_tc<BN, KIND>;
+  auto kfn = conv_gemm_pp<BN, KIND>;
+  if (!attr_set) {
+    cudaError_t e = cudaFuncSetAttribute(kfn, cudaFuncAttributeMaxDynamicSharedMemorySize, PPCfg<BN>::SMEM);
+    SEG_REQUIRE(e == cudaSuccess, "cudaFuncSetAttribute(smem=%d): %s", PPCfg<BN>::SMEM, cudaGetErrorString(e));
+    attr_set = true;
+  }
+  const int n_tiles = ceil_div(p.Ncols, BN);
+  const int64_t tiles = ceil_div64(p.M, BM) * n_tiles;
+  SEG_REQUIRE(tiles < (1ll << 31), "too many output tiles");
+  p.n_tiles = n_tiles;
+  p.tiles = (int)tiles;
+  const dim3 grid((unsigned)std::min<int64_t>(tiles, num_sms()));
+  launch_pdl(kfn, grid, dim3(NTHREADS), (size_t)PPCfg<BN>::SMEM, stream, p);
+  return check_launch("conv_gemm_pp");
+}
+
+template <int KIND>
+static int launch_pp_bn(int bn, TcParams& p, cudaStream_t stream) {
+  switch (bn) {
+    case 64: return launch_pp<64, KIND>(p, stream);
+    case 128: return launch_pp<128, KIND>(p, stream);
+  }
+  set_error("bad BN %d", bn);
+  return 1;
+}
+
+template <int BN>
+static int launch_wgrad(const TcParams& p, dim3 grid, cudaStream_t stream) {
+  static bool attr_set = false;
+  auto kfn = conv_gemm_wgrad<BN>;
   if (!attr_set) {
     cudaError_t e = cudaFuncSetAttribute(kfn, cudaFuncAttributeMaxDynamicSharedMemorySize, Cfg<BN>::SMEM);
     SEG_REQUIRE(e == cudaSuccess, "cudaFuncSetAttribute(smem=%d): %s", Cfg<BN>::SMEM, cudaGetErrorString(e));
     attr_set = true;
   }
   launch_pdl(kfn, grid, dim3(NTHREADS), (size_t)Cfg<BN>::SMEM, stream, p);
-  return check_launch("conv_gemm_tc");
-}
-
-template <int KIND>
-static int launch_bn(int bn, const TcParams& p, dim3 grid, cudaStream_t stream) {
+  return check_launch("conv_gemm_wgrad");
+}
+
+static int launch_wgrad_bn(int bn, const TcParams& p, dim3 grid, cudaStream_t stream) {
   switch (bn) {
-    case 64: return launch_kernel<64, KIND>(p, grid, stream);
-    case 128: return launch_kernel<128, KIND>(p, grid, stream);
-    case 256: return launch_kernel<256, KIND>(p, grid, stream);
+    case 64: return launch_wgrad<64>(p, grid, stream);
+    case 128: return launch_wgrad<128>(p, grid, stream);
+    case 256: return launch_wgrad<256>(p, grid, stream);
   }
   set_error("bad BN %d", bn);
   return 1;
 }
 
-static int pick_bn(int ncols) {
-  if (ncols <= 64) return 64;
-  if (ncols < 256) return 128;
-  const int waste = ceil_div(ncols, 256) * 256 - ncols;
-  return waste < 128 ? 256 : 128;
+static int pick_bn(int ncols, bool out_f32) { return (ncols <= 64 || out_f32) ? 64 : 128; }
+
+static int stat_rows_for(int ncols) {
+  if (ncols <= 64) return 32;
+  if (ncols < 256) return 64;
+  return ceil_div(ncols, 256) * 256 - ncols < 128 ? 128 : 64;
 }
 
 bool supported(const seg_conv_desc* d) {
@@ -506,8 +652,8 @@
     SEG_REQUIRE(4 * d->K <= sync->n_max, "conv fwd: 2*K = %d fp64 statistics exceed the SyncBN buffer (%d floats)", 2 * d->K, sync->n_max);
     p.sync = *sync;
   }
-  const int64_t m_tiles = ceil_div64(M, BM);
-  const int bn = pick_bn(d->K);
+  const int bn = pick_bn(d->K, y_dtype != SEG_DT_BF16);
+  p.stat_rows = stat_rows_for(d->K);
   if (is_pointwise(d)) {
     p.x_im2col = 0;
     if (make_map_2d(&p.mapA, x, M, d->C, d->ldx, BM)) return 1;
@@ -517,8 +663,7 @@
     if (make_map_im2col(&p.mapA, x, d->N, d->H, d->W, d->C, d->ldx, -d->pad, -d->pad, upper, upper, d->stride, BM)) return 1;
   }
   if (make_map_2d(&p.mapB, w, (int64_t)p.taps * d->K, d->C, d->C, bn)) return 1;
-  dim3 grid((unsigned)m_tiles, (unsigned)ceil_div(d->K, bn), 1);
-  return launch_bn<KIND_KK>(bn, p, grid, stream);
+  return launch_pp_bn<KIND_KK>(bn, p, stream);
 }
 
 static int floordiv(int a, int b) { return (a >= 0) ? a / b : -((-a + b - 1) / b); }
@@ -527,7 +672,7 @@
   SEG_REQUIRE(supported(d) && d->ldy % 8 == 0, "wgmma conv dgrad: unsupported shape (stride=%d K=%d ldy=%d)", d->stride,
               d->K, d->ldy);
   const int s = d->stride;
-  const int bn = pick_bn(d->C);
+  const int bn = pick_bn(d->C, false);
   for (int py = 0; py < s; ++py) {
     for (int px = 0; px < s; ++px) {
       const int Hs = (d->H - py + s - 1) / s, Ws = (d->W - px + s - 1) / s;
@@ -577,7 +722,7 @@
         p.opy = py;
         p.opx = px;
       }
-      const int64_t m_tiles = ceil_div64(M, BM);
+      p.stat_rows = BM;
       if (p.taps > 0) {
         const bool plain = (s == 1 && is_pointwise(d));
         if (plain) {
@@ -594,8 +739,7 @@
         if (make_map_2d(&p.mapA, w, (int64_t)d->R * d->S * d->K, d->C, d->C, BM)) return 1;
         if (make_map_2d(&p.mapB, w, (int64_t)d->R * d->S * d->K, d->C, d->C, 64)) return 1;
       }
-      dim3 grid((unsigned)m_tiles, (unsigned)ceil_div(d->C, bn), 1);
-      if (launch_bn<KIND_KM>(bn, p, grid, stream)) return 1;
+      if (launch_pp_bn<KIND_KM>(bn, p, stream)) return 1;
     }
   }
   return 0;
@@ -666,7 +810,7 @@
   }
   SEG_REQUIRE((unsigned)(p.taps * splits) <= 65535u, "wgrad grid.z too large");
   dim3 grid((unsigned)ceil_div(d->K, BM), (unsigned)ceil_div(d->C, bn), (unsigned)(p.taps * splits));
-  if (launch_bn<KIND_MM>(bn, p, grid, stream)) return 1;
+  if (launch_wgrad_bn(bn, p, grid, stream)) return 1;
   if (splits == 1) return 0;
   const int64_t n = (int64_t)p.taps * d->K * d->C;
   wgrad_split_reduce_kernel<<<(unsigned)std::min<int64_t>(ceil_div64(n, 256), (int64_t)num_sms() * 8), 256, 0, stream>>>(ws, splits, n, dw);
diff --git a/pytorch-segmentation_b200/csrc/seg_ptx.cuh b/pytorch-segmentation_b200/csrc/seg_ptx.cuh
--- a/pytorch-segmentation_b200/csrc/seg_ptx.cuh
+++ b/pytorch-segmentation_b200/csrc/seg_ptx.cuh
@@ -70,6 +70,17 @@
       : "memory");
 }
 
+template <int N>
+__device__ __forceinline__ void setmaxnreg_inc() { asm volatile("setmaxnreg.inc.sync.aligned.u32 %0;" ::"n"(N)); }
+template <int N>
+__device__ __forceinline__ void setmaxnreg_dec() { asm volatile("setmaxnreg.dec.sync.aligned.u32 %0;" ::"n"(N)); }
+__device__ __forceinline__ void named_sync(int id, int count) {
+  asm volatile("bar.sync %0, %1;" ::"r"(id), "r"(count) : "memory");
+}
+__device__ __forceinline__ void named_arrive(int id, int count) {
+  asm volatile("bar.arrive %0, %1;" ::"r"(id), "r"(count) : "memory");
+}
+
 __device__ __forceinline__ void wgmma_fence() { asm volatile("wgmma.fence.sync.aligned;" ::: "memory"); }
 __device__ __forceinline__ void wgmma_commit() { asm volatile("wgmma.commit_group.sync.aligned;" ::: "memory"); }
 template <int N>
```
